# fanliaoooo/xuanpolicy

Hardware: NVIDIA B200
Metric: PPO env-steps/s (higher is better)
Workload: dtype f32

## Files before the change

### include/xb200.h

```cpp
#ifndef XB200_H
#define XB200_H

#include <stdint.h>

#ifdef __cplusplus
extern "C" {
#endif

#define XB_VERSION 100
#define XB_OBS_STRIDE 4

#define XB_ENV_CARTPOLE 0
#define XB_ENV_PENDULUM 1
#define XB_ENV_MOUNTAINCAR 2
#define XB_ENV_ACROBOT 3
#define XB_ENV_MOUNTAINCAR_STACK4 4

#define XB_E_BADARG (-1)
#define XB_E_UNSUPPORTED (-2)
#define XB_E_DRIVER (-3)

#define XB_GAE_AUTO 0
#define XB_GAE_LDG 1
#define XB_GAE_TMA 2
// ... 113 lines not shown
int xb_dense_split_weights(const float* W, int N, int K, float* hi, float* lo, float* thi, float* tlo, int ldt,
                           int toff, xb_stream_t stream);
int xb_dense_split_weights2(const float* W0, float* hi0, float* lo0, const float* W1, float* hi1, float* lo1, int N, int K,
                            float* thi, float* tlo, xb_stream_t stream);
int xb_dense_fwd(const float* X, int64_t M, int K, const float* Whi, const float* Wlo, int N, const float* bias,
                 float slope, float* Y, const float* head_w, const float* head_b, int n_head, float* head_out,
                 int b_resident, xb_stream_t stream);
int xb_dense_wgrad_workspace_floats(int H_in);
int xb_mlp_backward_tail(const float* wgrad_ws, int H_out, int H_in, int n_sources, int nh0, int nh1, float* dW0, float* db0,
                         float* dw2_0, float* db2_0, float* dW1, float* db1, float* dw2_1, float* db2_1,
                         const float* trunk_ws, int trunk_parts, int obs_dim, float* dWt, float* dbt, const double* dls64,
                         float* dls32, int A, xb_stream_t stream);
int xb_mlp_backward_tail_norm(const float* wgrad_ws, int H_out, int H_in, int n_sources, int nh0, int nh1, float* dW0,
                              float* db0, float* dw2_0, float* db2_0, float* dW1, float* db1, float* dw2_1, float* db2_1,
                              const float* trunk_ws, int trunk_parts, int obs_dim, float* dWt, float* dbt,
                              const double* dls64, float* dls32, int A, double* norm_workspace, int64_t* step_dev,
                              float lr0, float lr_end_factor, int64_t lr_total_iters, float beta1, float beta2,
                              float max_norm, float grad_scale, float* lr_out, float* gnorm_out, xb_stream_t stream);
int xb_dense_wgrad(const float* Y0, const float* dout0, const float* w2_0, int nh0, const float* Y1, const float* dout1,
                   const float* w2_1, int nh1, const float* X, int64_t B, int H_out, int H_in, float slope,
                   float* workspace, float* dW0, float* db0, float* dw2_0, float* db2_0, float* dW1, float* db1,
                   float* dw2_1, float* db2_1, xb_stream_t stream);
int xb_dense_wgrad_bin(const uint32_t* signs, int sign_ld, const float* dout0, int nh0, const float* dout1, int nh1,
                       const float* X, int64_t B, int H_out, int H_in, float* workspace, xb_stream_t stream);
int xb_mlp_backward_tail_bin(const float* wgrad_ws, int H_out, int H_in, int n_sources, int nh0, int nh1, float* dW0,
                             float* db0, float* dw2_0, float* db2_0, float* dW1, float* db1, float* dw2_1, float* db2_1,
                             const float* trunk_ws, int trunk_parts, int obs_dim, float* dWt, float* dbt, const double* dls64,
                             float* dls32, int A, double* norm_workspace, int64_t* step_dev, float lr0, float lr_end_factor,
                             int64_t lr_total_iters, float beta1, float beta2, float max_norm, float grad_scale, float* lr_out,
                             float* gnorm_out, const float* W0, const float* b0, const float* w2_0, const float* W1,
                             const float* b1, const float* w2_1, float slope, xb_stream_t stream);
int xb_dense_fwd2(const float* X, int64_t M, int K, int N, float slope, const float* Whi0, const float* Wlo0,
                  const float* bias0, float* Y0, const float* head_w0, const float* head_b0, int n_head0, float* head_out0,
                  const float* Whi1, const float* Wlo1, const float* bias1, float* Y1, const float* head_w1,
                  const float* head_b1, int n_head1, float* head_out1, int b_resident, const float* prep_W0,
                  const float* prep_W1, float* prep_thi, float* prep_tlo, uint32_t* sign_out, xb_stream_t stream);
#define XB_FWD_WEIGHTS_STABLE 1
int xb_dense_fwd2_loss(const float* X, int64_t M, int K, int N, float slope, const float* Whi0, const float* Wlo0,
                       const float* bias0, float* Y0, const float* head_w0, const float* head_b0, int n_head0,
                       float* head_out0, const float* Whi1, const float* Wlo1, const float* bias1, float* Y1,
                       const float* head_w1, const float* head_b1, int n_head1, float* head_out1, int b_resident,
                       const float* scal, const double* adv_stats, int64_t adv_count, float clip_range, float vf_coef,
                       float ent_coef, float inv_batch, const float* logstd, float* dact, float* dv, double* loss_partials,
                       uint32_t* loss_ticket, double* scalars, double* dlogstd, const float* prep_W0, const float* prep_W1,
                       float* prep_thi, float* prep_tlo, uint32_t* sign_out, xb_stream_t stream);
int xb_mlp_fwd_from_obs_train(const float* obs, int ld, int obs_dim, const float* W0, const float* b0, int64_t M, int H,
                              float slope, const float* Whi0, const float* Wlo0, const float* bias0, float* Y0,
// ... 67 lines not shown
```

### xuanpolicy_b200/_lib.py

```python
import ctypes as C
import os

_PKG = os.path.dirname(os.path.abspath(__file__))
LIB_PATH = os.environ.get("XB200_LIB") or os.path.join(_PKG, "libxb200.so")

_i64, _i32, _f32, _f64, _u64, _vp = C.c_int64, C.c_int, C.c_float, C.c_double, C.c_uint64, C.c_void_p

SIGNATURES = {
    "xb_version": [],
    "xb_env_reset": [_i32, _vp, _vp, _vp, _vp, _vp, _i32, _i64, _vp],
    "xb_env_step": [_i32, _vp, _vp, _vp, _vp, _vp, _vp, _vp, _vp, _vp, _vp, _vp, _vp, _vp, _vp, _i32, _i64, _vp],
    "xb_rollout_step": [_i32, _vp, _vp, _vp, _u64, _vp, _u64, _vp, _vp, _vp, _vp, _vp, _vp, _vp, _vp, _vp, _vp, _vp, _vp, _vp,
                        _i32, _vp, _vp, _vp, _vp, _vp, _vp, _vp, _vp, _vp, _vp, _vp, _f32, _vp, _vp, _vp,
                        _vp, _vp, _i32, _f32, _vp, _vp, _vp, _f64, _i32, _vp, _vp, _vp, _i64, _vp],
    "xb_eval_step": [_i32, _vp, _vp, _vp, _vp, _vp, _vp, _vp, _vp, _vp, _vp, _i32, _vp, _i64, _vp, _vp, _vp, _i64, _vp, _vp,
                     _i32, _vp, _vp, _i64, _vp],
    "xb_sincos_f64": [_vp, _vp, _vp, _i64, _vp],
    "xb_store": [_vp, _vp, _i32, _i32, _vp, _vp, _vp, _vp, _vp, _vp, _vp, _vp, _vp, _vp, _vp, _vp, _vp, _f32, _i32, _i64, _vp],
    "xb_gae": [_vp, _vp, _vp, _vp, _vp, _vp, _vp, _vp, _vp, _i64, _i64, _f64, _f64, _i32, _i32, _vp],
    "xb_gather_obs": [_vp, _i64, _i64, _i64, _vp, _i32, _vp, _vp, _vp, _vp],
    "xb_gather_batch": [_vp, _i64, _i64, _i64, _vp, _i32, _vp, _i32, _vp, _vp, _vp, _vp, _vp, _vp, _vp, _vp, _vp, _vp,
                        _vp, _vp],
    "xb_normalize_adv": [_vp, _vp, _i64, _i64, _vp],
    "xb_ppo_loss_categorical": [_vp, _i64, _i64, _i64, _vp, _i32, _vp, _vp, _vp, _vp, _vp, _vp, _vp, _i64, _f32, _f32,
# ... 33 lines not shown
    "xb_dense_fwd2_loss": [_vp, _i64, _i32, _i32, _f32, _vp, _vp, _vp, _vp, _vp, _vp, _i32, _vp, _vp, _vp, _vp, _vp, _vp, _vp,
                           _i32, _vp, _i32, _vp, _vp, _i64, _f32, _f32, _f32, _f32, _vp, _vp, _vp, _vp, _vp, _vp, _vp, _vp, _vp, _vp,
                           _vp, _vp, _vp],
    "xb_mlp_fwd_from_obs": [_vp, _i32, _i32, _vp, _vp, _i64, _i32, _f32, _vp, _vp, _vp, _vp, _vp, _vp, _i32, _vp, _vp, _vp, _vp,
                            _vp, _vp, _vp, _i32, _vp, _vp, _vp, _i64, _f32, _i32, _vp],
    "xb_mlp_fwd_from_obs_train": [_vp, _i32, _i32, _vp, _vp, _i64, _i32, _f32, _vp, _vp, _vp, _vp, _vp, _vp, _i32, _vp, _vp, _vp,
                                  _vp, _vp, _vp, _vp, _i32, _vp, _vp, _vp, _vp, _i64, _f32, _f32, _f32, _f32, _vp, _vp, _vp, _vp,
                                  _vp, _vp, _vp, _vp, _vp, _vp, _vp, _vp, _vp],
    "xb_dense_dgrad": [_vp, _vp, _vp, _i32, _i32, _vp, _vp, _vp, _i32, _i32, _i64, _vp, _vp, _i32, _vp, _f32, _vp, _i32, _vp,
                       _vp, _vp],
    "xb_dense_wgrad_workspace_floats": [_i32],
    "xb_dense_wgrad": [_vp, _vp, _vp, _i32, _vp, _vp, _vp, _i32, _vp, _i64, _i32, _i32, _f32, _vp, _vp, _vp, _vp, _vp, _vp,
                       _vp, _vp, _vp, _vp],
    "xb_mlp_trunk_fwd": [_vp, _i32, _i32, _vp, _vp, _f32, _vp, _i64, _i32, _vp, _vp],
    "xb_mlp_trunk_wgrad_workspace_floats": [_i32, _i32],
    "xb_mlp_trunk_wgrad_parts": [],
    "xb_mlp_backward_tail": [_vp, _i32, _i32, _i32, _i32, _i32, _vp, _vp, _vp, _vp, _vp, _vp, _vp, _vp, _vp, _i32, _i32, _vp,
                             _vp, _vp, _vp, _i32, _vp],
    "xb_mlp_backward_tail_norm": [_vp, _i32, _i32, _i32, _i32, _i32, _vp, _vp, _vp, _vp, _vp, _vp, _vp, _vp, _vp, _i32, _i32,
                                  _vp, _vp, _vp, _vp, _i32, _vp, _vp, _f32, _f32, _i64, _f32, _f32, _f32, _f32, _vp, _vp, _vp],
    "xb_mlp_backward_tail_bin": [_vp, _i32, _i32, _i32, _i32, _i32, _vp, _vp, _vp, _vp, _vp, _vp, _vp, _vp, _vp, _i32, _i32,
                                 _vp, _vp, _vp, _vp, _i32, _vp, _vp, _f32, _f32, _i64, _f32, _f32, _f32, _f32, _vp, _vp,
                                 _vp, _vp, _vp, _vp, _vp, _vp, _f32, _vp],
    "xb_dense_wgrad_bin": [_vp, _i32, _vp, _i32, _vp, _i32, _vp, _i64, _i32, _i32, _vp, _vp],
    "xb_head3_fold": [_vp, _vp, _vp, _vp, _i32, _vp],
    "xb_head3_unfold_grads": [_vp, _vp, _i32, _vp],
    "xb_mlp_trunk_wgrad": [_vp, _vp, _i32, _i32, _vp, _vp, _vp, _i64, _i32, _vp],
    "xb_peer_stats_max": [],
    "xb_peer_alloc": [_vp, _i64],
    "xb_peer_free": [_vp],
    "xb_peer_export": [_vp, _vp],
    "xb_peer_import": [_vp, _vp],
    "xb_peer_close": [_vp],
    "xb_peer_allreduce_grad_norm": [_vp, _i32, _i32, _i64, _vp, _vp, _vp, _vp, _f32, _f32, _i64, _f32, _f32, _f32, _f32, _f32, _vp,
                                    _vp, _vp, _vp],
    "xb_adam_apply": [_vp, _vp, _vp, _vp, _i64, _f32, _f32, _f32, _f32, _vp, _vp],
    "xb_adam_apply_split": [_vp, _vp, _vp, _vp, _i64, _f32, _f32, _f32, _f32, _vp, _i64, _vp, _vp, _i64, _vp, _vp, _i32, _i32,
                            _vp, _vp, _vp],
    "xb_peer_allreduce_mean": [_vp, _i32, _i32, _i64, _vp, _vp, _vp, _vp],
    "xb_peer_allreduce_f64": [_vp, _i32, _i32, _i32, _i32, _vp, _vp, _vp],
    "xb_peer_allreduce_merge": [_vp, _i32, _i32, _vp, _i32, _i32, _vp, _vp, _vp, _vp, _i32, _vp, _vp, _vp],
    "xb_adv_stats_minibatches": [_vp, _i64, _i64, _i64, _i64, _vp, _i64, _vp, _vp],
    "xb_clip_adam_step": [_vp, _vp, _vp, _vp, _i64, _vp, _f32, _f32, _i64, _f32, _f32, _f32, _f32, _f32, _vp, _vp, _vp, _vp],
}

_lib = None

# ... 39 lines not shown
```

### xuanpolicy_b200/csrc/common.cuh

```cuda
#pragma once
#include <cuda_runtime.h>
#include <stdint.h>
#include <stdlib.h>

#include "../../include/xb200.h"

#define XB_LAUNCH_CHECK()                        \
    do {                                         \
        cudaError_t e__ = cudaGetLastError();    \
        if (e__ != cudaSuccess) return (int)e__; \
    } while (0)

#define XB_CUDA(call)                            \
    do {                                         \
        cudaError_t e__ = (call);                \
        if (e__ != cudaSuccess) return (int)e__; \
    } while (0)

namespace xb {

constexpr int kNumSMs = 148;

static inline int ceil_div_i64(int64_t a, int64_t b) { return (int)((a + b - 1) / b); }

static inline int grid_for(int64_t n, int block, int ctas_per_sm) {
    int64_t need = (n + block - 1) / block;
    int64_t cap = (int64_t)kNumSMs * ctas_per_sm;
    if (need < 1) need = 1;
    return (int)(need < cap ? need : cap);
}

__device__ __forceinline__ void pdl_wait() { asm volatile("griddepcontrol.wait;" ::: "memory"); }
__device__ __forceinline__ void pdl_trigger() { asm volatile("griddepcontrol.launch_dependents;" ::: "memory"); }

static inline bool pdl_enabled() {
    static const bool on = []() { const char* e = getenv("XB_PDL"); return !(e && e[0] == '0'); }();
    return on;
}

template <typename... KArgs, typename... Args>
static inline cudaError_t launch_pdl(void (*kern)(KArgs...), dim3 grid, dim3 block, size_t smem, cudaStream_t stream, bool pdl,
                                     Args&&... args) {
    cudaLaunchConfig_t cfg = {};
    cfg.gridDim = grid;
// ... 66 lines not shown
```

### xuanpolicy_b200/csrc/dense_tc.cu

```cuda
#include <stdlib.h>
#include <string.h>

#include "common.cuh"
#include "normalize.cuh"
#include "optim.cuh"
#include "sm100.cuh"

#ifdef XB_STEP_TS
extern unsigned long long* g_xb_step_ts;
#endif

namespace xb {
namespace dense {

using namespace sm100;

#ifdef XB_DENSE_TS
static long long* g_xb_ts_host = nullptr;
#define XB_TS(role, it, ev) do { if (p.ts && blockIdx.x == 0 && (it) < 64) p.ts[((role) * 64 + (it)) * 8 + (ev)] = clock64(); } while (0)
#else
#define XB_TS(role, it, ev) do { } while (0)
#endif

constexpr int BM = 128;
constexpr int BK = 32;
constexpr int kATile = BM * BK * 4;
constexpr int kOperandWarps = 8;
constexpr int kProducerWarp = 4 + kOperandWarps, kMmaWarp = kProducerWarp + 1;
constexpr int kThreads = (kMmaWarp + 1) * 32;
constexpr int kMiscBytes = 9216;
constexpr int kLossRedOff = 8704;
constexpr int kWMiscBytes = 15360;
constexpr int kMaxSmem = 232448;

enum { MODE_FWD = 0, MODE_DGRAD = 1 };

struct FusedLoss {
    const float4* scal;
    const double* adv_stats;
    double inv_adv_count;
    float clip_range, vf_coef, ent_coef, inv_batch;
    int gaussian;
    const float* logstd;
    float* dact;
    float* dv;
    double* partials;
    unsigned int* ticket;
    double* scalars;
    double* dlogstd;
};

struct KParams {
    FusedLoss loss;
    int64_t M;
    int KB;
// ... 1574 lines not shown
        "setp.ne.b32 c2, %11, 0;\n"
        "and.pred c2, c2, pe;\n"
        "@c2 tcgen05.commit.cta_group::1.mbarrier::arrive::one.shared::cluster.b64 [%11];\n"
        "selp.u32 %0, 1, 0, pn;\n"
        "}\n"
        : "=r"(ready)
        : "r"(d_tmem), "l"(da), "l"(db_hi), "l"(db_lo), "r"(idesc), "r"(accumulate_first), "r"(next_bar), "r"(next_par),
          "r"(commit0), "r"(commit1), "r"(commit2), "r"(elected)
        : "memory");
    return ready;
}

struct WBinParams {
    int64_t B;
    int n_jobs, halves, H_out;
    int stages, lo_bufs;
    const float* dout[2];
    int nh[2];
    const uint32_t* signs;
    int sign_ld;
    float* part;
    float* head_part;
    float* db2_part;
};

template <int HIN>
__global__ void __launch_bounds__(kThreads, 1)
    dense_wgrad_bin_kernel(const __grid_constant__ CUtensorMap map_x, const WBinParams p) {
    constexpr int NBX = HIN / 32;
    constexpr int kBox = 32 * 128;
    constexpr int kStage = 4 * kBox + NBX * kBox;
    constexpr int kLo = NBX * kBox;
    constexpr int kTmemCols = HIN;
    constexpr int kGroups = HIN == 128 ? 3 : 2;
    constexpr int kOw = 4 * kGroups;
    constexpr uint32_t kIdescMain = umma_idesc_tf32(128, HIN, 1, 1);
    extern __shared__ unsigned char smem_raw[];
    const uint32_t base = (smem_u32(smem_raw) + 1023u) & ~1023u;
    const int S = p.stages, L = p.lo_bufs;
    const uint32_t ring = base, lo_ring = ring + (uint32_t)S * kStage, misc = lo_ring + (uint32_t)L * kLo;
    const uint32_t bar_full = misc, bar_conv = misc + 64, bar_empty = misc + 128, bar_loempty = misc + 192;
    const uint32_t bar_tfull = misc + 256, tmem_slot = misc + 264;
    unsigned char* misc_ptr = smem_raw + (misc - smem_u32(smem_raw));
    float* sf = reinterpret_cast<float*>(misc_ptr + 2048);

    const int warp = threadIdx.x >> 5, lane = threadIdx.x & 31;
    const int job = blockIdx.x % p.n_jobs, q = blockIdx.x / p.n_jobs;
    const int cj = (gridDim.x - job + p.n_jobs - 1) / p.n_jobs;
    const int src = job / p.halves, m0 = (job % p.halves) * 128;
    const int64_t nblk = (p.B + 31) / 32;
    const int64_t blk0 = nblk * q / cj, blk1 = nblk * (q + 1) / cj;
    const int nkb = (int)(blk1 - blk0);

    if (threadIdx.x == 0) {
        for (int s = 0; s < S; ++s) {
            mbar_init(bar_full + 8 * s, 1);
            mbar_init(bar_conv + 8 * s, kOperandWarps / 2);
            mbar_init(bar_empty + 8 * s, 1);
        }
        for (int j = 0; j < L; ++j) mbar_init(bar_loempty + 8 * j, 1);
        mbar_init(bar_tfull, 1);
        mbar_fence_init();
    }
    if (warp == kMmaWarp) tmem_alloc<kTmemCols>(tmem_slot);
    pdl_wait();
    pdl_trigger();
    tc_fence_before();
    __syncthreads();
    tc_fence_after();
    uint32_t tmem_base;
    asm volatile("ld.shared.u32 %0, [%1];" : "=r"(tmem_base) : "r"(tmem_slot));

    if (warp == kProducerWarp) {
        const uint32_t elected = elect_one_pred();
        if (lane == 0) tma_prefetch_desc(&map_x);
        __syncwarp();
        uint32_t s = 0, ph = 0;
        for (int it = 0; it < nkb; ++it) {
            mbar_wait(bar_empty + 8 * s, ph ^ 1);
            const uint32_t st = ring + s * kStage;
            mbar_arrive_expect_tx_if(elected, bar_full + 8 * s, NBX * kBox);
            const int row = (int)((blk0 + it) * 32);
#pragma unroll
            for (int g = 0; g < NBX; ++g) tma_load_2d_if(elected, st + (4 + g) * kBox, &map_x, g * 32, row, bar_full + 8 * s);
            if (++s == (uint32_t)S) { s = 0; ph ^= 1; }
        }
    } else if (warp == kMmaWarp) {
        const uint32_t elected = elect_one_pred();
        const uint32_t tmem_base_u = __reduce_max_sync(0xffffffffu, tmem_base);
        uint32_t s = 0, ph = 0, j = 0, ready = 0;
        for (int it = 0; it < nkb; ++it) {
            if (!ready) mbar_wait(bar_conv + 8 * s, ph);
            tc_fence_after();
            const uint32_t a = ring + s * kStage, b_hi = a + 4 * kBox, b_lo = lo_ring + j * kLo;
            const uint32_t ns = s + 1 == (uint32_t)S ? 0 : s + 1, nph = s + 1 == (uint32_t)S ? ph ^ 1 : ph;
            ready = ss_kblock_mn_bin(tmem_base_u, umma_desc_sw128_base32(a, kBox, 512), umma_desc_sw128_base32(b_hi, kBox, 512),
// ... 658 lines not shown
    return backward_tail_impl(wgrad_ws, H_out, H_in, n_sources, nh0, nh1, dW0, db0, dw2_0, db2_0, dW1, db1, dw2_1, db2_1,
                              trunk_ws, trunk_parts, obs_dim, dWt, dbt, dls64, dls32, A, nullptr, nullptr, none, nullptr,
                              nullptr, (cudaStream_t)stream);
}

extern "C" int xb_mlp_backward_tail_norm(const float* wgrad_ws, int H_out, int H_in, int n_sources, int nh0, int nh1,
                                         float* dW0, float* db0, float* dw2_0, float* db2_0, float* dW1, float* db1,
                                         float* dw2_1, float* db2_1, const float* trunk_ws, int trunk_parts, int obs_dim,
                                         float* dWt, float* dbt, const double* dls64, float* dls32, int A,
                                         double* norm_workspace, int64_t* step_dev, float lr0, float lr_end_factor,
                                         int64_t lr_total_iters, float beta1, float beta2, float max_norm, float grad_scale,
                                         float* lr_out, float* gnorm_out, xb_stream_t stream) {
    if (!norm_workspace || !step_dev || !trunk_ws) return XB_E_BADARG;
    xb::AdamHyper h{lr0, lr_end_factor, beta1, beta2, 0.0f, max_norm, grad_scale, lr_total_iters};
    return backward_tail_impl(wgrad_ws, H_out, H_in, n_sources, nh0, nh1, dW0, db0, dw2_0, db2_0, dW1, db1, dw2_1, db2_1,
                              trunk_ws, trunk_parts, obs_dim, dWt, dbt, dls64, dls32, A, norm_workspace, step_dev, h, lr_out,
                              gnorm_out, (cudaStream_t)stream);
}


template <int HIN>
static int launch_wgrad_bin(const CUtensorMap& mx, WBinParams p, int grid, cudaStream_t s) {
    const int stage = (4 + HIN / 32) * 4096, lo = (HIN / 32) * 4096;
    const int avail = kMaxSmem - 1024 - kWMiscBytes;
    int L = 2, S = (avail - L * lo) / stage;
    if (S < 2) return XB_E_UNSUPPORTED;
    if (S > 6) S = 6;
    if ((avail - S * stage) / lo >= 3) L = 3;
    p.stages = S;
    p.lo_bufs = L;
    const int smem = 1024 + S * stage + L * lo + kWMiscBytes;
    auto kern = dense_wgrad_bin_kernel<HIN>;
    XB_CUDA(cudaFuncSetAttribute(kern, cudaFuncAttributeMaxDynamicSharedMemorySize, kMaxSmem));
    XB_CUDA(launch_pdl(kern, dim3(grid), dim3(kThreads), (size_t)smem, s, true, mx, p));
    XB_LAUNCH_CHECK();
    return 0;
}

extern "C" int xb_dense_wgrad_bin(const uint32_t* signs, int sign_ld, const float* dout0, int nh0, const float* dout1, int nh1,
                                  const float* X, int64_t B, int H_out, int H_in, float* workspace, xb_stream_t stream) {
    if (!signs || !dout0 || !X || !workspace || B <= 0) return XB_E_BADARG;
    if ((H_out != 128 && H_out != 256) || (H_in != 128 && H_in != 256) || nh0 < 1 || nh0 > 2) return XB_E_UNSUPPORTED;
    if (dout1 && (nh1 < 1 || nh1 > 2)) return XB_E_BADARG;
    const int n_src = dout1 ? 2 : 1;
    if (sign_ld < n_src * (H_out / 32)) return XB_E_BADARG;
    if (!al16(X) || !al16(workspace)) return XB_E_UNSUPPORTED;
    CUtensorMap mx;
    if (!xb_make_map_f32_2d(&mx, X, B, H_in, H_in, 32, 32, 2)) return XB_E_DRIVER;
    WBinParams p{};
    p.B = B;
    p.halves = H_out / 128;
    p.n_jobs = n_src * p.halves;
    p.H_out = H_out;
    p.dout[0] = dout0; p.nh[0] = nh0;
    p.dout[1] = dout1; p.nh[1] = dout1 ? nh1 : 0;
    p.signs = signs;
    p.sign_ld = sign_ld;
    const int grid = kNumSMs;
    p.part = workspace;
    p.head_part = workspace + (int64_t)grid * 128 * (H_in + 4);
    p.db2_part = p.head_part + (int64_t)grid * 256;
    return H_in == 128 ? launch_wgrad_bin<128>(mx, p, grid, (cudaStream_t)stream) : launch_wgrad_bin<256>(mx, p, grid, (cudaStream_t)stream);
}

extern "C" int xb_mlp_backward_tail_bin(const float* wgrad_ws, int H_out, int H_in, int n_sources, int nh0, int nh1,
                                        float* dW0, float* db0, float* dw2_0, float* db2_0, float* dW1, float* db1,
                                        float* dw2_1, float* db2_1, const float* trunk_ws, int trunk_parts, int obs_dim,
                                        float* dWt, float* dbt, const double* dls64, float* dls32, int A,
                                        double* norm_workspace, int64_t* step_dev, float lr0, float lr_end_factor,
                                        int64_t lr_total_iters, float beta1, float beta2, float max_norm, float grad_scale,
                                        float* lr_out, float* gnorm_out, const float* W0, const float* b0, const float* w2_0,
                                        const float* W1, const float* b1, const float* w2_1, float slope, xb_stream_t stream) {
    if (!W0 || !b0 || !w2_0 || (n_sources == 2 && (!W1 || !b1 || !w2_1))) return XB_E_BADARG;
    if (norm_workspace && (!step_dev || !trunk_ws)) return XB_E_BADARG;
    xb::AdamHyper h{lr0, lr_end_factor, beta1, beta2, 0.0f, max_norm, grad_scale, lr_total_iters};
    if (!norm_workspace) h.grad_scale = 1.0f;
    BinArgs bin{1, slope, {W0, W1}, {b0, b1}, {w2_0, w2_1}};
    return backward_tail_impl(wgrad_ws, H_out, H_in, n_sources, nh0, nh1, dW0, db0, dw2_0, db2_0, dW1, db1, dw2_1, db2_1,
                              trunk_ws, trunk_parts, obs_dim, dWt, dbt, dls64, dls32, A, norm_workspace, step_dev, h, lr_out,
                              gnorm_out, (cudaStream_t)stream, bin);
}


extern "C" int xb_mlp_fwd_from_obs_train(const float* obs, int ld, int obs_dim, const float* W0, const float* b0, int64_t M, int H,
// ... 29 lines not shown
```

### xuanpolicy_b200/csrc/mlp_trunk.cu

```cuda
#include "common.cuh"

namespace xb {

constexpr int kMaxObs = 8;

template <int OBS>
__global__ void __launch_bounds__(256) trunk_fwd_kernel(const float* __restrict__ obs, int ld, const float* __restrict__ W0,
                                                        const float* __restrict__ b0, float slope, float4* __restrict__ h1,
                                                        int64_t B, int H, uint32_t* __restrict__ h1_signs) {
    const int tpr = H >> 2;
    const int rows_per_block = blockDim.x / tpr;
    const int q = threadIdx.x % tpr, slot = threadIdx.x / tpr;
    if (slot >= rows_per_block) return;
    const int lane = threadIdx.x & 31;
    float w[4][OBS], bias[4];
#pragma unroll
    for (int e = 0; e < 4; ++e) {
        bias[e] = b0[4 * q + e];
#pragma unroll
        for (int i = 0; i < OBS; ++i) w[e][i] = W0[(4 * q + e) * OBS + i];
    }
    for (int64_t b = (int64_t)blockIdx.x * rows_per_block + slot; b < B; b += (int64_t)gridDim.x * rows_per_block) {
        float x[OBS];
#pragma unroll
// ... 65 lines not shown
    for (int k = threadIdx.x; k < n_out; k += blockDim.x) {
        float s = 0.f;
        for (int r = 0; r < rows_per_block; ++r) s += red[r * n_out + k];
        partial[(int64_t)blockIdx.x * n_out + k] = s;
    }
}

__global__ void __launch_bounds__(256) trunk_wgrad_reduce_kernel(const float* __restrict__ partial, int n_blocks, int H,
                                                                 int OBS, float* __restrict__ dW0,
                                                                 float* __restrict__ db0) {
    const int k = blockIdx.x * (blockDim.x >> 5) + (threadIdx.x >> 5), lane = threadIdx.x & 31;
    const int n_out = H * (OBS + 1);
    if (k >= n_out) return;
    float s = 0.f;
    for (int p = lane; p < n_blocks; p += 32) s += partial[(int64_t)p * n_out + k];
    s = warp_sum(s);
    if (lane == 0) {
        const int n = k / (OBS + 1), i = k % (OBS + 1);
        if (i < OBS) dW0[n * OBS + i] = s;
        else db0[n] = s;
    }
}

constexpr int kTrunkBlocks = 3 * kNumSMs;

}

using namespace xb;

#define XB_OBS_SWITCH(OBS, CALL)        \
    switch (OBS) {                      \
        case 1: { constexpr int O = 1; CALL; } break; \
        case 2: { constexpr int O = 2; CALL; } break; \
        case 3: { constexpr int O = 3; CALL; } break; \
        case 4: { constexpr int O = 4; CALL; } break; \
        case 5: { constexpr int O = 5; CALL; } break; \
        case 6: { constexpr int O = 6; CALL; } break; \
        case 7: { constexpr int O = 7; CALL; } break; \
        case 8: { constexpr int O = 8; CALL; } break; \
        default: return XB_E_UNSUPPORTED;             \
    }

static inline bool trunk_shape_ok(int obs_dim, int H) {
    return obs_dim >= 1 && obs_dim <= kMaxObs && H % 4 == 0 && H >= 4 && 256 % (H / 4) == 0;
}

extern "C" int xb_mlp_trunk_fwd(const float* obs, int ld, int obs_dim, const float* W0, const float* b0, float slope,
                                float* h1, int64_t B, int H, uint32_t* h1_signs, xb_stream_t stream) {
// ... 66 lines not shown
```

### xuanpolicy_b200/csrc/sm100.cuh

```cuda
#pragma once
#include <cuda.h>
#include <cuda_runtime.h>
#include <stdint.h>

namespace xb {
namespace sm100 {

__device__ __forceinline__ uint32_t smem_u32(const void* ptr) { return (uint32_t)__cvta_generic_to_shared(ptr); }

__device__ __forceinline__ void mbar_init(uint32_t bar, uint32_t count) {
    asm volatile("mbarrier.init.shared::cta.b64 [%0], %1;" ::"r"(bar), "r"(count) : "memory");
}
__device__ __forceinline__ void mbar_fence_init() { asm volatile("fence.mbarrier_init.release.cluster;" ::: "memory"); }
__device__ __forceinline__ void mbar_arrive_expect_tx(uint32_t bar, uint32_t bytes) {
    asm volatile("mbarrier.arrive.expect_tx.shared::cta.b64 _, [%0], %1;" ::"r"(bar), "r"(bytes) : "memory");
}
__device__ __forceinline__ void mbar_arrive(uint32_t bar) {
    asm volatile("mbarrier.arrive.shared::cta.b64 _, [%0];" ::"r"(bar) : "memory");
}
__device__ __forceinline__ uint32_t elect_one_pred() {
    uint32_t e;
    asm volatile(
        "{\n"
        ".reg .pred p;\n"
// ... 24 lines not shown
        "cp.async.bulk.tensor.2d.shared::cluster.global.mbarrier::complete_tx::bytes [%0], [%1, {%2, %3}], [%4];"
        ::"r"(smem_dst), "l"((uint64_t)map), "r"(c0), "r"(c1), "r"(bar)
        : "memory");
}
__device__ __forceinline__ void tma_load_2d_if(uint32_t elected, uint32_t smem_dst, const CUtensorMap* map, int c0, int c1,
                                               uint32_t bar) {
    asm volatile(
        "{\n"
        ".reg .pred pe;\n"
        "setp.ne.b32 pe, %5, 0;\n"
        "@pe cp.async.bulk.tensor.2d.shared::cluster.global.mbarrier::complete_tx::bytes [%0], [%1, {%2, %3}], [%4];\n"
        "}\n" ::"r"(smem_dst), "l"((uint64_t)map), "r"(c0), "r"(c1), "r"(bar), "r"(elected)
        : "memory");
}
__device__ __forceinline__ void mbar_arrive_expect_tx_if(uint32_t elected, uint32_t bar, uint32_t bytes) {
    asm volatile(
        "{\n"
        ".reg .pred pe;\n"
        "setp.ne.b32 pe, %2, 0;\n"
        "@pe mbarrier.arrive.expect_tx.shared::cta.b64 _, [%0], %1;\n"
        "}\n" ::"r"(bar), "r"(bytes), "r"(elected)
        : "memory");
}
__device__ __forceinline__ void tma_store_2d_commit_if(uint32_t elected, const CUtensorMap* map, uint32_t smem_src, int c0,
                                                       int c1) {
    asm volatile(
        "{\n"
        ".reg .pred pe;\n"
        "setp.ne.b32 pe, %4, 0;\n"
        "@pe cp.async.bulk.tensor.2d.global.shared::cta.bulk_group [%0, {%1, %2}], [%3];\n"
        "@pe cp.async.bulk.commit_group;\n"
        "}\n" ::"l"((uint64_t)map), "r"(c0), "r"(c1), "r"(smem_src), "r"(elected)
        : "memory");
}
__device__ __forceinline__ void tma_store_2d(const CUtensorMap* map, uint32_t smem_src, int c0, int c1) {
    asm volatile("cp.async.bulk.tensor.2d.global.shared::cta.bulk_group [%0, {%1, %2}], [%3];" ::"l"((uint64_t)map),
                 "r"(c0), "r"(c1), "r"(smem_src)
                 : "memory");
}
__device__ __forceinline__ void tma_prefetch_desc(const CUtensorMap* map) {
    asm volatile("prefetch.tensormap [%0];" ::"l"((uint64_t)map) : "memory");
}
__device__ __forceinline__ void fence_proxy_async_smem() { asm volatile("fence.proxy.async.shared::cta;" ::: "memory"); }

template <int kCols>
__device__ __forceinline__ void tmem_alloc(uint32_t smem_result_addr) {
// ... 134 lines not shown
```

### xuanpolicy_b200/fused_mlp.py

```python
import os

import torch
import torch.nn as nn

from . import ops


def _stack(seq):
    return list(seq) if isinstance(seq, nn.Sequential) else None


class _OutParams:

    def __init__(self, logits=None, mu=None, std=None):
        self._logits, self._mu, self._std = logits, mu, std

    def get_param(self):
        return self._logits if self._logits is not None else (self._mu, self._std)


class FusedActorCritic:
    MIN_ROWS = 2048

    @staticmethod
# ... 28 lines not shown
                if not t.is_cuda or t.dtype != torch.float32:
                    return None
        return dict(l0=l0, la1=la1, la2=la2, lc1=lc1, lc2=lc2, H=H, obs_dim=l0.in_features, A=la2.out_features,
                    slope=float(a0.negative_slope), gaussian=hasattr(policy.actor, "logstd"))

    def __init__(self, policy):
        pl = self.plan(policy)
        if pl is None:
            raise ValueError("policy structure not supported by the fused dense kernels")
        self.policy = policy
        self.__dict__.update(pl)
        dev = self.l0.weight.device
        self.device = dev
        H = self.H
        z = lambda *s: torch.zeros(*s, dtype=torch.float32, device=dev)
        self.wa_hi, self.wa_lo, self.wc_hi, self.wc_lo = z(H, H), z(H, H), z(H, H), z(H, H)
        self.wt_hi, self.wt_lo = z(H, 2 * H), z(H, 2 * H)
        self.wtm_hi, self.wtm_lo = z(H, 2 * H), z(H, 2 * H)
        self.mask_dgrad = os.environ.get("XB_MASK_DGRAD", "1") != "0"
        self.sign_bits = os.environ.get("XB_SIGN_BITS", "1") != "0"
        self.sign_dgrad = self.sign_bits and H == 128
        self.bin_wgrad = self.sign_bits and os.environ.get("XB_BIN_WGRAD", "1") != "0"
        self._bin_now = False
        self.h1_signs = self.sign_dgrad and os.environ.get("XB_H1_SIGNS", "0") == "1"
        self._mask_ready = False
        self.fold3 = (not self.gaussian) and self.A == 3
        self.nh_a = 2 if self.fold3 else self.A
        self.w2f, self.b2f = (z(2, H), z(2)) if self.fold3 else (None, None)
        self.ws_wgrad = ops.dense_wgrad_workspace(H, dev)
        self.ws_trunk = ops.mlp_trunk_wgrad_workspace(self.obs_dim, H, dev)
        self._buf = {}
        self._last = None
        self.norm_sink, self.norm_done = None, False
        self.splits_fresh = False
        self._loss_partials = torch.zeros(148 * 8, dtype=torch.float64, device=dev)
        self._loss_ticket = torch.zeros(1, dtype=torch.int32, device=dev)
        self.fork_wgrad = os.environ.get("XB_FORK_WGRAD", "0") == "1"
        self._side = None

    def _head_a(self):
        return (self.w2f, self.b2f) if self.fold3 else (self.la2.weight.data, self.la2.bias.data)

    def fold_head(self):
        if self.fold3:
            ops.head3_fold(self.la2.weight.data, self.la2.bias.data, self.w2f, self.b2f)

# ... 44 lines not shown
            return
        if loss is None:
            ops.dense_fwd2(b["h1"], self.slope, l0, l1, prep=prep, sign_out=b["signs"])
            if self.fold3:
                b["act"][:, :2].copy_(b["act2"])
            return
        ops.dense_fwd2_loss(b["h1"], self.slope, l0, l1, loss["scal"], loss["adv_stats"], loss["adv_count"],
                            loss["clip_range"], loss["vf_coef"], loss["ent_coef"], loss["inv_batch"], loss["logstd"],
                            b["dact"], b["dv"], self._loss_partials, self._loss_ticket, loss["scalars"], loss["dlogstd"],
                            prep=prep, sign_out=b["signs"])

    def stage_dgrad(self, b, dact, dv2, softmax_pair=False):
        assert b.get("y_valid", True) or (self.sign_dgrad and b.get("signs") is not None), "forward(keep_y=False) needs the sign-word dgrad"
        if self._mask_ready and (self.A == 1 or (self.A == 2 and softmax_pair)):
            ops.dense_dgrad(b["ya"], dact, self.la2.weight.data, b["yc"], dv2, self.lc2.weight.data, self.wtm_hi, self.wtm_lo,
                            b["h1"], self.slope, b["dz1"], wt_form=1, signs=b["signs"], h1_signs=b.get("h1s"))
            return
        ops.dense_dgrad(b["ya"], dact, self._head_a()[0], b["yc"], dv2, self.lc2.weight.data, self.wt_hi, self.wt_lo,
                        b["h1"], self.slope, b["dz1"], signs=b["signs"], h1_signs=b.get("h1s"))

    def _rank1(self, softmax_pair):
        return (not self.fold3) and (self.A == 1 or (self.A == 2 and softmax_pair))

    def stage_wgrad(self, b, dact, dv2, softmax_pair=False):
        self._bin_now = self.bin_wgrad and self._rank1(softmax_pair) and b.get("signs") is not None
        if self._bin_now:
            ops.dense_wgrad_bin(b["signs"], dact, self.A, dv2, 1, b["h1"], self.H, self.ws_wgrad)
            return
        assert b.get("y_valid", True), "forward(keep_y=False) needs the binary-form wgrad (rank-1 head gradients)"
        ops.dense_wgrad(b["ya"], dact, self._head_a()[0], b["yc"], dv2, self.lc2.weight.data, b["h1"], self.slope,
                        self.ws_wgrad, None, None, None, None)

    def stage_trunk_wgrad(self, obs, b):
        ops.mlp_trunk_wgrad(b["dz1"], obs, self.ws_trunk, None, None)

    def stage_tail(self, dls64=None, dls32=None):
        g = lambda p: p.grad
        norm, self.norm_done = None, False
        if self.norm_sink is not None and not self.fold3 and (not self.gaussian or dls64 is not None):
            fl, max_norm = self.norm_sink
            norm = (fl.workspace, fl.step, fl.lr0, fl.end_factor, fl.total_iters, fl.beta1, fl.beta2, max_norm, 1.0, fl.lr,
                    fl.gnorm)
            self.norm_done = True
        bin_form = None
        if self._bin_now:
            bin_form = (self.la1.weight.data, self.la1.bias.data, self.la2.weight.data, self.lc1.weight.data, self.lc1.bias.data,
                        self.lc2.weight.data, self.slope)
        ops.mlp_backward_tail(self.ws_wgrad, self.H, self.H, self.nh_a, 1,
                              (g(self.la1.weight), g(self.la1.bias), g(self.la2.weight), g(self.la2.bias)),
                              (g(self.lc1.weight), g(self.lc1.bias), g(self.lc2.weight), g(self.lc2.bias)),
                              self.ws_trunk, self.obs_dim, g(self.l0.weight), g(self.l0.bias), dls64, dls32, norm=norm,
                              bin_form=bin_form)
        if self.fold3:
            ops.head3_unfold_grads(g(self.la2.weight), g(self.la2.bias))
# ... 37 lines not shown
    def backward(self, dact, dv, dls64=None, dls32=None, softmax_pair=False):
        obs, b = self._last
        B = obs.shape[0]
        if b["dz1"] is None:
            b["dz1"] = torch.empty(B, self.H, dtype=torch.float32, device=self.device)
        dv2 = dv.reshape(B, 1)
        if self.fold3:
            if "dact2" not in b:
                b["dact2"] = torch.empty(B, 2, dtype=torch.float32, device=self.device)
            b["dact2"].copy_(dact[:, :2])
            dact = b["dact2"]
        if self.fork_wgrad:
            cur = torch.cuda.current_stream(self.device)
            if self._side is None:
                self._side = torch.cuda.Stream(device=self.device)
            self._side.wait_stream(cur)
            self.stage_dgrad(b, dact, dv2, softmax_pair)
            with torch.cuda.stream(self._side):
                self.stage_wgrad(b, dact, dv2, softmax_pair)
            self.stage_trunk_wgrad(obs, b)
            cur.wait_stream(self._side)
        else:
            self.stage_dgrad(b, dact, dv2, softmax_pair)
            self.stage_wgrad(b, dact, dv2, softmax_pair)
            self.stage_trunk_wgrad(obs, b)
        self.stage_tail(dls64, dls32)
```

### xuanpolicy_b200/ops.py

```python
import torch

from . import _lib

ENV_KINDS = {"CartPole-v1": 0, "Pendulum-v1": 1, "gym:MountainCar-v0": 2, "Acrobot-v1": 3, "MountainCar-v0": 4}
GAE_VARIANTS = {"auto": 0, "ldg": 1, "tma": 2}


def _p(t, dtype=None):
    if t is None:
        return None
    if not t.is_cuda:
        raise _lib.XB200Error("xb200 kernels take CUDA tensors (got a %s tensor); there is no CPU path" % t.device)
    if not t.is_contiguous():
        raise _lib.XB200Error("xb200 kernels take contiguous tensors")
    if dtype is not None and t.dtype != dtype:
        raise _lib.XB200Error("expected dtype %s, got %s" % (dtype, t.dtype))
    return t.data_ptr()


def _stream():
    return torch.cuda.current_stream().cuda_stream


F32, F64, I64, I32, U8 = torch.float32, torch.float64, torch.int64, torch.int32, torch.uint8
# ... 384 lines not shown
    B, H_out = y0.shape
    _lib.call("xb_dense_wgrad", _p(y0, F32), _p(dout0, F32), _p(w2_0, F32), w2_0.shape[0], _p(y1, F32), _p(dout1, F32),
              _p(w2_1, F32), w2_1.shape[0] if w2_1 is not None else 0, _p(x, F32), B, H_out, x.shape[1], float(slope),
              _p(workspace, F32), _p(dW0, F32), _p(db0, F32), _p(dw2_0, F32), _p(db2_0, F32), _p(dW1, F32), _p(db1, F32),
              _p(dw2_1, F32), _p(db2_1, F32), _stream())


def mlp_trunk_fwd(obs, w0, b0, slope, h1, h1_signs=None):
    ptr, ld = _rows_ld(obs)
    _lib.call("xb_mlp_trunk_fwd", ptr, ld, obs.shape[1], _p(w0, F32), _p(b0, F32), float(slope), _p(h1, F32),
              obs.shape[0], w0.shape[0], _p(h1_signs, I32), _stream())


def mlp_trunk_wgrad_workspace(obs_dim, h, device):
    return torch.empty(_lib.load().xb_mlp_trunk_wgrad_workspace_floats(int(obs_dim), int(h)), dtype=F32, device=device)


def mlp_trunk_wgrad(dz1, obs, workspace, dw0, db0):
    ptr, ld = _rows_ld(obs)
    _lib.call("xb_mlp_trunk_wgrad", _p(dz1, F32), ptr, ld, obs.shape[1], _p(workspace, F32), _p(dw0, F32), _p(db0, F32),
              obs.shape[0], dz1.shape[1], _stream())


def dense_wgrad_bin(signs, dout0, nh0, dout1, nh1, x, h_out, workspace):
    B, h_in = x.shape
    _lib.call("xb_dense_wgrad_bin", _p(signs, I32), signs.shape[1], _p(dout0, F32), nh0, _p(dout1, F32), nh1, _p(x, F32), B,
              h_out, h_in, _p(workspace, F32), _stream())


def mlp_backward_tail(wgrad_ws, h_out, h_in, nh0, nh1, grads0, grads1, trunk_ws, obs_dim, dwt, dbt, dls64=None, dls32=None,
                      norm=None, bin_form=None):
    parts = _lib.load().xb_mlp_trunk_wgrad_parts()
    args = [_p(wgrad_ws, F32), h_out, h_in, 2 if grads1 is not None else 1, nh0, nh1,
            *[_p(g, F32) for g in grads0], *([_p(g, F32) for g in grads1] if grads1 is not None else [None] * 4),
            _p(trunk_ws, F32), parts, obs_dim, _p(dwt, F32), _p(dbt, F32), _p(dls64, F64), _p(dls32, F32),
            dls64.numel() if dls64 is not None else 0]
    if bin_form is not None:
        ws, step_dev, lr0, end_factor, total_iters, beta1, beta2, max_norm, grad_scale, lr_out, gnorm_out = \
            norm if norm is not None else (None, None, 0.0, 1.0, 1, 0.9, 0.999, 0.0, 1.0, None, None)
        W0, b0, w2_0, W1, b1, w2_1, slope = bin_form
        _lib.call("xb_mlp_backward_tail_bin", *args, _p(ws, F64), _p(step_dev, I64), float(lr0), float(end_factor),
                  int(total_iters), float(beta1), float(beta2), float(max_norm), float(grad_scale), _p(lr_out, F32),
                  _p(gnorm_out, F32), _p(W0, F32), _p(b0, F32), _p(w2_0, F32), _p(W1, F32), _p(b1, F32), _p(w2_1, F32),
                  float(slope), _stream())
    elif norm is None:
        _lib.call("xb_mlp_backward_tail", *args, _stream())
    else:
        ws, step_dev, lr0, end_factor, total_iters, beta1, beta2, max_norm, grad_scale, lr_out, gnorm_out = norm
        _lib.call("xb_mlp_backward_tail_norm", *args, _p(ws, F64), _p(step_dev, I64), float(lr0), float(end_factor),
                  int(total_iters), float(beta1), float(beta2), float(max_norm), float(grad_scale), _p(lr_out, F32),
# ... 10 lines not shown
```

Measured before the change: 50.08 million.

## Fuse trunk weight-gradient into binary wgrad kernel via extra warps

Adds two extra warps to the binary-form dense wgrad kernel (H_in=128) that compute the first-layer trunk weight gradient from dz1 and obs. dz1 rows are streamed with 1D bulk async copies into a per-warp shared-memory ring guarded by mbarriers. The per-block partial sums are written in the same layout the separate trunk wgrad kernel used, so the tail reduction can consume them unchanged. This removes one kernel launch and lets the trunk reduction overlap the tensor-core wgrad, at the cost of shared memory taken from the main pipeline stages and more threads per block.

```diff
diff --git a/include/xb200.h b/include/xb200.h
--- a/include/xb200.h
+++ b/include/xb200.h
@@ -159,7 +159,8 @@
                    float* workspace, float* dW0, float* db0, float* dw2_0, float* db2_0, float* dW1, float* db1,
                    float* dw2_1, float* db2_1, xb_stream_t stream);
 int xb_dense_wgrad_bin(const uint32_t* signs, int sign_ld, const float* dout0, int nh0, const float* dout1, int nh1,
-                       const float* X, int64_t B, int H_out, int H_in, float* workspace, xb_stream_t stream);
+                       const float* X, int64_t B, int H_out, int H_in, float* workspace, const float* dz1, const float* obs,
+                       int ld, int obs_dim, float* trunk_ws, xb_stream_t stream);
 int xb_mlp_backward_tail_bin(const float* wgrad_ws, int H_out, int H_in, int n_sources, int nh0, int nh1, float* dW0,
                              float* db0, float* dw2_0, float* db2_0, float* dW1, float* db1, float* dw2_1, float* db2_1,
                              const float* trunk_ws, int trunk_parts, int obs_dim, float* dWt, float* dbt, const double* dls64,
diff --git a/xuanpolicy_b200/_lib.py b/xuanpolicy_b200/_lib.py
--- a/xuanpolicy_b200/_lib.py
+++ b/xuanpolicy_b200/_lib.py
@@ -79,7 +79,7 @@
     "xb_mlp_backward_tail_bin": [_vp, _i32, _i32, _i32, _i32, _i32, _vp, _vp, _vp, _vp, _vp, _vp, _vp, _vp, _vp, _i32, _i32,
                                  _vp, _vp, _vp, _vp, _i32, _vp, _vp, _f32, _f32, _i64, _f32, _f32, _f32, _f32, _vp, _vp,
                                  _vp, _vp, _vp, _vp, _vp, _vp, _f32, _vp],
-    "xb_dense_wgrad_bin": [_vp, _i32, _vp, _i32, _vp, _i32, _vp, _i64, _i32, _i32, _vp, _vp],
+    "xb_dense_wgrad_bin": [_vp, _i32, _vp, _i32, _vp, _i32, _vp, _i64, _i32, _i32, _vp, _vp, _vp, _i32, _i32, _vp, _vp],
     "xb_head3_fold": [_vp, _vp, _vp, _vp, _i32, _vp],
     "xb_head3_unfold_grads": [_vp, _vp, _i32, _vp],
     "xb_mlp_trunk_wgrad": [_vp, _vp, _i32, _i32, _vp, _vp, _vp, _i64, _i32, _vp],
diff --git a/xuanpolicy_b200/csrc/common.cuh b/xuanpolicy_b200/csrc/common.cuh
--- a/xuanpolicy_b200/csrc/common.cuh
+++ b/xuanpolicy_b200/csrc/common.cuh
@@ -20,6 +20,7 @@
 namespace xb {
 
 constexpr int kNumSMs = 148;
+constexpr int kTrunkBlocks = 3 * kNumSMs;
 
 static inline int ceil_div_i64(int64_t a, int64_t b) { return (int)((a + b - 1) / b); }
 
diff --git a/xuanpolicy_b200/csrc/dense_tc.cu b/xuanpolicy_b200/csrc/dense_tc.cu
--- a/xuanpolicy_b200/csrc/dense_tc.cu
+++ b/xuanpolicy_b200/csrc/dense_tc.cu
@@ -31,6 +31,10 @@
 constexpr int kMiscBytes = 9216;
 constexpr int kLossRedOff = 8704;
 constexpr int kWMiscBytes = 15360;
+constexpr int kTrunkWarps = 2, kTrunkStages = 4, kTrunkRows = 8;
+constexpr int kTrunkChunk = kTrunkRows * 128 * 4;
+constexpr int kTrunkRing = kTrunkWarps * kTrunkStages * kTrunkChunk;
+constexpr int kTrunkBarOff = 512;
 constexpr int kMaxSmem = 232448;
 
 enum { MODE_FWD = 0, MODE_DGRAD = 1 };
@@ -1651,10 +1655,120 @@
     float* part;
     float* head_part;
     float* db2_part;
+    const float* dz1;
+    const float* obs;
+    int obs_ld, obs_dim;
+    float* trunk_part;
 };
 
 template <int HIN>
-__global__ void __launch_bounds__(kThreads, 1)
+constexpr int bin_threads() { return HIN == 128 ? kThreads + 32 * kTrunkWarps : kThreads; }
+
+template <int OBS>
+__device__ __forceinline__ void trunk_wgrad_blocks(const WBinParams& p, uint32_t ring, uint32_t bars, int g, int n_warps) {
+    constexpr int64_t kTrunkStep = (int64_t)kTrunkBlocks * 8;
+    const int lane = threadIdx.x & 31;
+    const int nsets = 8 * ((kTrunkBlocks - g + n_warps - 1) / n_warps);
+    auto first = [&](int set) { return (int64_t)(g + (set >> 3) * n_warps) * 8 + (set & 7); };
+    auto nrows = [&](int set) { const int64_t f = first(set); return f < p.B ? (int)((p.B - f + kTrunkStep - 1) / kTrunkStep) : 0; };
+    int total = 0;
+    for (int set = 0; set < nsets; ++set) total += nrows(set);
+    auto advance = [&](int& set, int64_t& row) {
+        row += kTrunkStep;
+        if (row >= p.B) row = first(++set);
+    };
+    const int nch = (total + kTrunkRows - 1) / kTrunkRows;
+    const uint32_t elected = elect_one_pred();
+    int pset = 0;
+    int64_t prow = first(0);
+    auto issue = [&](int k) {
+        const int n = min(kTrunkRows, total - k * kTrunkRows);
+        const uint32_t bar = bars + 8 * (k % kTrunkStages), st = ring + (k % kTrunkStages) * kTrunkChunk;
+        mbar_arrive_expect_tx_if(elected, bar, (uint32_t)n * 512u);
+        for (int r = 0; r < n; ++r) {
+            bulk_load_1d_if(elected, st + r * 512, p.dz1 + prow * 128, 512u, bar);
+            advance(pset, prow);
+        }
+    };
+    for (int k = 0; k < kTrunkStages && k < nch; ++k) issue(k);
+    float acc[4][OBS + 1], sum[4][OBS + 1];
+#pragma unroll
+    for (int e = 0; e < 4; ++e)
+#pragma unroll
+        for (int i = 0; i <= OBS; ++i) acc[e][i] = sum[e][i] = 0.f;
+    float xn[OBS];
+    int oset = 0;
+    int64_t orow = first(0);
+    auto load_obs = [&]() {
+        int64_t mine = -1;
+#pragma unroll
+        for (int r = 0; r < kTrunkRows; ++r) {
+            if (lane == r && oset < nsets && orow < p.B) mine = orow;
+            advance(oset, orow);
+        }
+#pragma unroll
+        for (int i = 0; i < OBS; ++i) xn[i] = mine >= 0 ? __ldg(p.obs + mine * p.obs_ld + i) : 0.f;
+    };
+    auto store = [&](int set) {
+        float* out = p.trunk_part + (int64_t)(g + (set >> 3) * n_warps) * (128 * (OBS + 1));
+#pragma unroll
+        for (int e = 0; e < 4; ++e)
+#pragma unroll
+            for (int i = 0; i <= OBS; ++i) {
+                out[(4 * lane + e) * (OBS + 1) + i] = sum[e][i];
+                sum[e][i] = 0.f;
+            }
+    };
+    int set = 0, left = nsets > 0 ? nrows(0) : 0;
+    load_obs();
+    for (int k = 0; k < nch; ++k) {
+        float x[OBS];
+#pragma unroll
+        for (int i = 0; i < OBS; ++i) x[i] = xn[i];
+        load_obs();
+        const int rows = min(kTrunkRows, total - k * kTrunkRows);
+        mbar_wait(bars + 8 * (k % kTrunkStages), (k / kTrunkStages) & 1);
+        const uint32_t st = ring + (k % kTrunkStages) * kTrunkChunk + lane * 16;
+#pragma unroll
+        for (int r = 0; r < kTrunkRows; ++r) {
+            if (r < rows) {
+                const float4 d = lds128(st + r * 512);
+                const float dv[4] = {d.x, d.y, d.z, d.w};
+                float xr[OBS];
+#pragma unroll
+                for (int i = 0; i < OBS; ++i) xr[i] = __shfl_sync(0xffffffffu, x[i], r);
+#pragma unroll
+                for (int e = 0; e < 4; ++e) {
+#pragma unroll
+                    for (int i = 0; i < OBS; ++i) acc[e][i] += dv[e] * xr[i];
+                    acc[e][OBS] += dv[e];
+                }
+                if (--left == 0) {
+#pragma unroll
+                    for (int e = 0; e < 4; ++e)
+#pragma unroll
+                        for (int i = 0; i <= OBS; ++i) {
+                            sum[e][i] += acc[e][i];
+                            acc[e][i] = 0.f;
+                        }
+                    if ((set & 7) == 7) store(set);
+                    ++set;
+                    left = set < nsets ? nrows(set) : 0;
+                }
+            }
+        }
+        if (k + kTrunkStages < nch) {
+            __syncwarp();
+            fence_proxy_async_smem();
+            issue(k + kTrunkStages);
+        }
+    }
+    for (; set < nsets; ++set)
+        if ((set & 7) == 7) store(set);
+}
+
+template <int HIN>
+__global__ void __launch_bounds__(bin_threads<HIN>(), 1)
     dense_wgrad_bin_kernel(const __grid_constant__ CUtensorMap map_x, const WBinParams p) {
     constexpr int NBX = HIN / 32;
     constexpr int kBox = 32 * 128;
@@ -1689,6 +1803,8 @@
         }
         for (int j = 0; j < L; ++j) mbar_init(bar_loempty + 8 * j, 1);
         mbar_init(bar_tfull, 1);
+        if (HIN == 128 && p.dz1)
+            for (int s = 0; s < kTrunkWarps * kTrunkStages; ++s) mbar_init(misc + kTrunkBarOff + 8 * s, 1);
         mbar_fence_init();
     }
     if (warp == kMmaWarp) tmem_alloc<kTmemCols>(tmem_slot);
@@ -1700,7 +1816,22 @@
     uint32_t tmem_base;
     asm volatile("ld.shared.u32 %0, [%1];" : "=r"(tmem_base) : "r"(tmem_slot));
 
-    if (warp == kProducerWarp) {
+    if (warp > kMmaWarp) {
+        if constexpr (HIN == 128) {
+            if (p.dz1) {
+                const int tw = warp - kMmaWarp - 1;
+                const uint32_t ring = misc + kWMiscBytes + tw * (kTrunkStages * kTrunkChunk);
+                const uint32_t bars = misc + kTrunkBarOff + tw * (8 * kTrunkStages);
+                const int g = tw * gridDim.x + blockIdx.x, n_warps = kTrunkWarps * gridDim.x;
+                switch (p.obs_dim) {
+                    case 1: trunk_wgrad_blocks<1>(p, ring, bars, g, n_warps); break;
+                    case 2: trunk_wgrad_blocks<2>(p, ring, bars, g, n_warps); break;
+                    case 3: trunk_wgrad_blocks<3>(p, ring, bars, g, n_warps); break;
+                    default: trunk_wgrad_blocks<4>(p, ring, bars, g, n_warps); break;
+                }
+            }
+        }
+    } else if (warp == kProducerWarp) {
         const uint32_t elected = elect_one_pred();
         if (lane == 0) tma_prefetch_desc(&map_x);
         __syncwarp();
@@ -2405,29 +2536,33 @@
 template <int HIN>
 static int launch_wgrad_bin(const CUtensorMap& mx, WBinParams p, int grid, cudaStream_t s) {
     const int stage = (4 + HIN / 32) * 4096, lo = (HIN / 32) * 4096;
-    const int avail = kMaxSmem - 1024 - kWMiscBytes;
+    const int trunk = p.dz1 ? kTrunkRing : 0;
+    const int avail = kMaxSmem - 1024 - kWMiscBytes - trunk;
     int L = 2, S = (avail - L * lo) / stage;
     if (S < 2) return XB_E_UNSUPPORTED;
     if (S > 6) S = 6;
     if ((avail - S * stage) / lo >= 3) L = 3;
     p.stages = S;
     p.lo_bufs = L;
-    const int smem = 1024 + S * stage + L * lo + kWMiscBytes;
+    const int smem = 1024 + S * stage + L * lo + kWMiscBytes + trunk;
     auto kern = dense_wgrad_bin_kernel<HIN>;
     XB_CUDA(cudaFuncSetAttribute(kern, cudaFuncAttributeMaxDynamicSharedMemorySize, kMaxSmem));
-    XB_CUDA(launch_pdl(kern, dim3(grid), dim3(kThreads), (size_t)smem, s, true, mx, p));
+    XB_CUDA(launch_pdl(kern, dim3(grid), dim3(bin_threads<HIN>()), (size_t)smem, s, true, mx, p));
     XB_LAUNCH_CHECK();
     return 0;
 }
 
 extern "C" int xb_dense_wgrad_bin(const uint32_t* signs, int sign_ld, const float* dout0, int nh0, const float* dout1, int nh1,
-                                  const float* X, int64_t B, int H_out, int H_in, float* workspace, xb_stream_t stream) {
+                                  const float* X, int64_t B, int H_out, int H_in, float* workspace, const float* dz1,
+                                  const float* obs, int ld, int obs_dim, float* trunk_ws, xb_stream_t stream) {
     if (!signs || !dout0 || !X || !workspace || B <= 0) return XB_E_BADARG;
     if ((H_out != 128 && H_out != 256) || (H_in != 128 && H_in != 256) || nh0 < 1 || nh0 > 2) return XB_E_UNSUPPORTED;
     if (dout1 && (nh1 < 1 || nh1 > 2)) return XB_E_BADARG;
     const int n_src = dout1 ? 2 : 1;
     if (sign_ld < n_src * (H_out / 32)) return XB_E_BADARG;
     if (!al16(X) || !al16(workspace)) return XB_E_UNSUPPORTED;
+    if (dz1 && (!obs || !trunk_ws || obs_dim < 1 || ld < obs_dim)) return XB_E_BADARG;
+    if (dz1 && (H_in != 128 || obs_dim > 4 || !al16(dz1))) return XB_E_UNSUPPORTED;
     CUtensorMap mx;
     if (!xb_make_map_f32_2d(&mx, X, B, H_in, H_in, 32, 32, 2)) return XB_E_DRIVER;
     WBinParams p{};
@@ -2443,6 +2578,11 @@
     p.part = workspace;
     p.head_part = workspace + (int64_t)grid * 128 * (H_in + 4);
     p.db2_part = p.head_part + (int64_t)grid * 256;
+    p.dz1 = dz1;
+    p.obs = obs;
+    p.obs_ld = ld;
+    p.obs_dim = obs_dim;
+    p.trunk_part = trunk_ws;
     return H_in == 128 ? launch_wgrad_bin<128>(mx, p, grid, (cudaStream_t)stream) : launch_wgrad_bin<256>(mx, p, grid, (cudaStream_t)stream);
 }
 
diff --git a/xuanpolicy_b200/csrc/mlp_trunk.cu b/xuanpolicy_b200/csrc/mlp_trunk.cu
--- a/xuanpolicy_b200/csrc/mlp_trunk.cu
+++ b/xuanpolicy_b200/csrc/mlp_trunk.cu
@@ -111,8 +111,6 @@
     }
 }
 
-constexpr int kTrunkBlocks = 3 * kNumSMs;
-
 }
 
 using namespace xb;
diff --git a/xuanpolicy_b200/csrc/sm100.cuh b/xuanpolicy_b200/csrc/sm100.cuh
--- a/xuanpolicy_b200/csrc/sm100.cuh
+++ b/xuanpolicy_b200/csrc/sm100.cuh
@@ -70,6 +70,16 @@
         "}\n" ::"r"(bar), "r"(bytes), "r"(elected)
         : "memory");
 }
+__device__ __forceinline__ void bulk_load_1d_if(uint32_t elected, uint32_t smem_dst, const void* src, uint32_t bytes,
+                                                uint32_t bar) {
+    asm volatile(
+        "{\n"
+        ".reg .pred pe;\n"
+        "setp.ne.b32 pe, %4, 0;\n"
+        "@pe cp.async.bulk.shared::cluster.global.mbarrier::complete_tx::bytes [%0], [%1], %2, [%3];\n"
+        "}\n" ::"r"(smem_dst), "l"((uint64_t)src), "r"(bytes), "r"(bar), "r"(elected)
+        : "memory");
+}
 __device__ __forceinline__ void tma_store_2d_commit_if(uint32_t elected, const CUtensorMap* map, uint32_t smem_src, int c0,
                                                        int c1) {
     asm volatile(
diff --git a/xuanpolicy_b200/fused_mlp.py b/xuanpolicy_b200/fused_mlp.py
--- a/xuanpolicy_b200/fused_mlp.py
+++ b/xuanpolicy_b200/fused_mlp.py
@@ -74,6 +74,7 @@
         self.sign_dgrad = self.sign_bits and H == 128
         self.bin_wgrad = self.sign_bits and os.environ.get("XB_BIN_WGRAD", "1") != "0"
         self._bin_now = False
+        self.trunk_in_wgrad = H == 128 and self.obs_dim <= 4 and os.environ.get("XB_TRUNK_IN_WGRAD", "1") != "0"
         self.h1_signs = self.sign_dgrad and os.environ.get("XB_H1_SIGNS", "0") == "1"
         self._mask_ready = False
         self.fold3 = (not self.gaussian) and self.A == 3
@@ -164,14 +165,17 @@
     def _rank1(self, softmax_pair):
         return (not self.fold3) and (self.A == 1 or (self.A == 2 and softmax_pair))
 
-    def stage_wgrad(self, b, dact, dv2, softmax_pair=False):
+    def stage_wgrad(self, b, dact, dv2, softmax_pair=False, obs=None):
         self._bin_now = self.bin_wgrad and self._rank1(softmax_pair) and b.get("signs") is not None
         if self._bin_now:
-            ops.dense_wgrad_bin(b["signs"], dact, self.A, dv2, 1, b["h1"], self.H, self.ws_wgrad)
-            return
+            trunk = obs is not None and self.trunk_in_wgrad
+            ops.dense_wgrad_bin(b["signs"], dact, self.A, dv2, 1, b["h1"], self.H, self.ws_wgrad,
+                                *((b["dz1"], obs, self.ws_trunk) if trunk else ()))
+            return trunk
         assert b.get("y_valid", True), "forward(keep_y=False) needs the binary-form wgrad (rank-1 head gradients)"
         ops.dense_wgrad(b["ya"], dact, self._head_a()[0], b["yc"], dv2, self.lc2.weight.data, b["h1"], self.slope,
                         self.ws_wgrad, None, None, None, None)
+        return False
 
     def stage_trunk_wgrad(self, obs, b):
         ops.mlp_trunk_wgrad(b["dz1"], obs, self.ws_trunk, None, None)
@@ -255,6 +259,6 @@
             cur.wait_stream(self._side)
         else:
             self.stage_dgrad(b, dact, dv2, softmax_pair)
-            self.stage_wgrad(b, dact, dv2, softmax_pair)
-            self.stage_trunk_wgrad(obs, b)
+            if not self.stage_wgrad(b, dact, dv2, softmax_pair, obs=obs):
+                self.stage_trunk_wgrad(obs, b)
         self.stage_tail(dls64, dls32)
diff --git a/xuanpolicy_b200/ops.py b/xuanpolicy_b200/ops.py
--- a/xuanpolicy_b200/ops.py
+++ b/xuanpolicy_b200/ops.py
@@ -430,10 +430,12 @@
               obs.shape[0], dz1.shape[1], _stream())
 
 
-def dense_wgrad_bin(signs, dout0, nh0, dout1, nh1, x, h_out, workspace):
+def dense_wgrad_bin(signs, dout0, nh0, dout1, nh1, x, h_out, workspace, dz1=None, obs=None, trunk_ws=None):
     B, h_in = x.shape
+    ptr, ld = _rows_ld(obs) if obs is not None else (None, 0)
     _lib.call("xb_dense_wgrad_bin", _p(signs, I32), signs.shape[1], _p(dout0, F32), nh0, _p(dout1, F32), nh1, _p(x, F32), B,
-              h_out, h_in, _p(workspace, F32), _stream())
+              h_out, h_in, _p(workspace, F32), _p(dz1, F32), ptr, ld, obs.shape[1] if obs is not None else 0,
+              _p(trunk_ws, F32), _stream())
 
 
 def mlp_backward_tail(wgrad_ws, h_out, h_in, nh0, nh1, grads0, grads1, trunk_ws, obs_dim, dwt, dbt, dls64=None, dls32=None,
```

Result: slower. 41.73 million, median of 6 (-16.7%).
